# Justin900429/autonomous_driving_with_diffusion_model

Hardware: AMD Instinct MI355X
Metric: denoising-steps/sec (higher is better)
Workload: dtype f32

## Files before the change

autonomous_driving_with_diffusion_model_amd/_lib.py:

```python
from __future__ import annotations

import ctypes as C
import os
from typing import Optional, Sequence

import torch

_HERE = os.path.dirname(os.path.abspath(__file__))
LIB_PATH = os.environ.get("ADX_LIB") or os.path.join(_HERE, "libadx.so")

c_f32p = C.POINTER(C.c_float)
i32, i64, f32, vp = C.c_int32, C.c_int64, C.c_float, C.c_void_p


class TConvDesc(C.Structure):
    _fields_ = [("kind", i32), ("taps", i32), ("stride", i32), ("pad", i32), ("c0", i32), ("c1", i32),
                ("cout", i32), ("lin", i32), ("lout", i32), ("groups", i32), ("eps", f32), ("w_layout", i32),
                ("w_flip", i32), ("exact", i32), ("lin_valid", i32), ("lout_valid", i32)]


class TConvIO(C.Structure):
    _fields_ = [("x0", vp), ("x0_sb", i64), ("x0_sc", i64), ("x0_sl", i64),
                ("x1", vp), ("x1_sb", i64), ("x1_sc", i64), ("x1_sl", i64),
                ("packed_w", vp), ("bias", vp), ("gamma", vp), ("beta", vp),
# ... 121 lines not shown
    "adx_conv2d_packed_bytes": (C.c_size_t, [C.POINTER(Conv2dDesc)]),
    "adx_conv2d_pack": (i32, [C.POINTER(Conv2dDesc), vp, vp, vp]),
    "adx_conv2d_forward": (i32, [C.POINTER(Conv2dDesc), vp, vp, vp, vp, vp, vp, i32, i32, i32, i32, vp]),
    "adx_conv2d_cells_supported": (i32, [C.POINTER(Conv2dDesc), i32, i32, i32]),
    "adx_conv2d_forward_cells": (i32, [C.POINTER(Conv2dDesc), vp, vp, vp, vp, vp, vp, i32, i32, i32, i32, i32, vp]),
    "adx_conv2d_stem_pool": (i32, [vp, i32, vp, vp, vp, vp, vp, vp, i32, i32, i32, i32, vp]),
    "adx_conv2d_wgrad_scratch_bytes": (C.c_size_t, []),
    "adx_conv2d_wgrad": (i32, [C.POINTER(Conv2dDesc), vp, vp, vp, i32, i32, i32, vp, vp]),
    "adx_conv2d_wgrad_ex": (i32, [C.POINTER(Conv2dDesc), vp, vp, vp, i32, i32, i32, vp, i32, vp]),
    "adx_conv2d_wgrad_cells": (i32, [C.POINTER(Conv2dDesc), vp, vp, vp, vp, i32, i32, i32, vp, vp]),
    "adx_trajpred_create": (i32, [i32, C.POINTER(vp)]),
    "adx_trajpred_destroy": (None, [vp]),
    "adx_trajpred_num_params": (i32, [vp]),
    "adx_trajpred_packed_bytes": (C.c_size_t, [vp]),
    "adx_trajpred_scratch_bytes": (C.c_size_t, [vp, i32, i32]),
    "adx_trajpred_set_scratch": (i32, [vp, vp, C.c_size_t]),
    "adx_trajpred_pack": (i32, [vp, C.POINTER(vp), i32, vp, vp, vp]),
    "adx_trajpred_forward": (i32, [vp, vp, vp, i64, i64, vp, vp, i32, i32, vp]),
    "adx_trajpred_backward": (i32, [vp, vp, vp, i64, i64, vp, vp, vp, i32, i32, vp]),
    "adx_trajpred_backward_params": (i32, [vp, vp, vp, i64, i64, vp, vp, vp, vp, vp, i32, i32, C.c_float, C.c_uint64, vp]),
    "adx_trajpred_forward_train": (i32, [vp, vp, vp, i64, i64, vp, vp, i32, i32, C.c_float, C.c_uint64, vp]),
    "adx_trajpred_param_offsets": (i32, [vp, C.POINTER(i64), i32]),
    "adx_guided_output": (i32, [vp, vp, vp, vp, vp, f32, f32, vp, vp, i32, i32, vp]),
    "adx_optim_chunk": (i32, []),
    "adx_adamw_ema_step": (i32, [vp, vp, vp, i32, f32, f32, f32, f32, f32, i32, f32, i32, i32, vp]),
    "adx_adamw_ema_step_scaled": (i32, [vp, vp, vp, i32, f32, f32, f32, f32, f32, i32, f32, i32, i32, f32, vp]),
    "adx_image_normalize": (i32, [vp, vp, i32, i32, i32, C.POINTER(C.c_float), C.POINTER(C.c_float), vp]),
    "adx_probe_mfma_fp16": (i32, [vp, vp, i32, i32, C.POINTER(C.c_double), vp]),
    "adx_probe_mfma_fp16_16x16x32": (i32, [vp, vp, i32, i32, C.POINTER(C.c_double), vp]),
    "adx_image_augment": (i32, [vp, vp, i32, i32, i32, vp, vp, vp, vp, i32, vp]),
    "adx_ddim_step": (i32, [C.POINTER(StepCoef), vp, vp, vp, vp, vp, vp, vp, i32, i32, i32, vp]),
    "adx_ddpm_step": (i32, [C.POINTER(StepCoef), vp, vp, vp, vp, vp, vp, vp, i32, i32, i32, vp]),
    "adx_ddim_step_rng": (i32, [C.POINTER(StepCoef), vp, vp, vp, i32, i64, vp, vp, vp, vp, i32, i32, i32, vp]),
    "adx_ddpm_step_rng": (i32, [C.POINTER(StepCoef), vp, vp, vp, i32, i64, vp, vp, vp, vp, i32, i32, i32, vp]),
    "adx_dpm_step": (i32, [C.POINTER(DpmCoef), vp, vp, vp, vp, vp, i32, i32, i32, vp]),
    "adx_traj_select": (i32, [C.POINTER(SelectCfg), vp, vp, vp, vp, vp, vp]),
    "adx_control_state_bytes": (C.c_size_t, [i32, i32, i32]),
    "adx_control_step": (i32, [C.POINTER(ControlCfg), vp, vp, vp, vp, vp, vp]),
    "adx_control_reset": (i32, [vp, i32, i32, i32, vp, vp]),
    "adx_noise_normal": (i32, [vp, i32, i64, vp, i64, vp]),
    "adx_noise_words": (i32, [vp, i32, i64, vp, i64, vp]),
    "adx_noise_advance": (i32, [vp, vp]),
    "adx_warm_init": (i32, [vp, i32, vp, vp, i32, i32, i32, i32, f32, f32, vp, i64, i32, vp]),
    "adx_add_noise": (i32, [vp, vp, vp, vp, vp, i32, vp, i32, i32, i32, i32, vp]),
}

_LAZY_SIGS = {
    "adx_conv2d_pack_ds": (i32, [i32, i32, vp, vp, vp]),
    "adx_conv2d_block_s2_cells": (i32, [i32, i32, vp, vp, vp, vp, vp, vp, vp, vp, vp, i32, i32, i32, i32, vp]),
    "adx_ddim_step_pin": (i32, [C.POINTER(StepCoef), vp, vp, vp, vp, i32, i64, C.POINTER(PinDesc), vp, vp, i32, i32, i32, vp]),
    "adx_ddpm_step_pin": (i32, [C.POINTER(StepCoef), vp, vp, vp, vp, i32, i64, C.POINTER(PinDesc), vp, vp, i32, i32, i32, vp]),
    "adx_dpm_step_pin": (i32, [C.POINTER(DpmCoef), vp, vp, vp, vp, i32, i64, C.POINTER(PinDesc), vp, vp, i32, i32, i32, vp]),
    "adx_pin_apply": (i32, [vp, C.POINTER(PinDesc), vp, i64, i32, i32, i32, vp]),
}

EXPORTED_SYMBOLS = tuple(_SIGS) + tuple(_LAZY_SIGS)

_lib: Optional[C.CDLL] = None


class AdxError(RuntimeError):
    pass


class AdxRangeError(AdxError):

    def __init__(self, groups):
        self.groups = list(groups)
        super().__init__(f"values outside the fp16 range of the split kernels (|x| >= 65504 or NaN) in {', '.join(self.groups)}; "
                         "ADX_CHECK_RANGE=1 names the first tensor, ADX_CONV_EXACT=1 runs the perception pass on the exact-fp32 kernels")


def lib() -> C.CDLL:
    global _lib
    if _lib is None:
        if not os.path.exists(LIB_PATH):
            raise AdxError(
                f"{LIB_PATH} not found: the HIP extension is not built. Run `python -c 'import __graft_entry__ as g; "
                f"g.build()'` (or autonomous_driving_with_diffusion_model_amd/csrc/build.sh). There is no CPU fallback.")
        handle = C.CDLL(LIB_PATH)
        for name, (res, args) in _SIGS.items():
            fn = getattr(handle, name)
            fn.restype = res
            fn.argtypes = args
        _lib = handle
    return _lib


def lazy(name: str):
    handle = lib()
    res, args = _LAZY_SIGS[name]
    try:
        fn = getattr(handle, name)
    except AttributeError:
        raise AdxError(f"{LIB_PATH} does not export {name} (a library built from older sources?)") from None
    fn.restype = res
    fn.argtypes = args
    return fn


class NativeTape:

    def __init__(self, create, destroy, what: str):
        import weakref
        h = vp()
        check(create(C.byref(h)), what)
# ... 54 lines not shown
```

autonomous_driving_with_diffusion_model_amd/csrc/conv2d.hip:

```cpp
#include <stdlib.h>

#include <vector>

#include "adx_common.h"
#include "conv2d_internal.h"

namespace adx {

constexpr int kCoutT = 64;
constexpr size_t kMaxLds = 96 * 1024;

template <int STRIDE, int K, int ROWS, int CCH = 16>
__global__ void __launch_bounds__(256) conv2d_kernel(const Conv2dArgs a) {
  constexpr int TH = 4 * ROWS;
  constexpr int CC = (K == 7) ? 4 : CCH;
  constexpr int PH = (TH - 1) * STRIDE + K;
  constexpr int PW = (kTileW - 1) * STRIDE + K;
  constexpr int PLANE = PH * PW;
  constexpr int NP = CC * PLANE;
  constexpr int PITEMS = (NP + 255) / 256;
  constexpr int NTAPS = K * K;
  constexpr int NW4 = NTAPS * CC * (kCoutT / 4);
  constexpr int WITEMS = (NW4 + 255) / 256;
  extern __shared__ __attribute__((aligned(16))) float smem[];
// ... 430 lines not shown
  else if (L.stride == 2 && L.k == 7) conv2d_kernel<2, 7, 1><<<g, blk, lds, s>>>(a);
  else if (L.stride == 1 && L.k == 1) conv2d_kernel<1, 1, 1><<<g, blk, lds, s>>>(a);
  else {
    set_error("conv2d: no kernel for k=%d stride=%d (ResNet-34 uses 3x3 s1, 3x3 s2, 1x1 s2, 7x7 s2)", L.k, L.stride);
    return ADX_ERR_INVALID;
  }
  ADX_LAUNCH_CHECK();
  return ADX_OK;
}

}

using namespace adx;

static int spec_from_desc(const adx_conv2d_desc* d, ConvSpec* L) {
  ADX_REQUIRE(d != nullptr, "conv2d: null descriptor");
  ADX_REQUIRE(d->cin >= 1 && d->cout >= 64 && d->cout % kCoutT == 0, "conv2d: cout %d must be a multiple of %d", d->cout,
              kCoutT);
  ADX_REQUIRE(d->k >= 1 && d->k <= 7 && (d->stride == 1 || d->stride == 2) && d->pad >= 0 && d->pad <= 3,
              "conv2d: unsupported k/stride/pad %d/%d/%d", d->k, d->stride, d->pad);
  memset(L, 0, sizeof(*L));
  L->cin = d->cin; L->cout = d->cout; L->k = d->k; L->stride = d->stride; L->pad = d->pad;
  L->cc = d->cin >= 16 ? 16 : 4;
  L->cin_pad = round_up(d->cin, L->cc);
  return ADX_OK;
}

extern "C" {

size_t adx_conv2d_packed_bytes(const adx_conv2d_desc* d) {
  ConvSpec L;
  if (spec_from_desc(d, &L) != ADX_OK) return 0;
  return sizeof(float) * (conv2d_hs_eligible(L) ? conv2d_packed_floats(L) : (size_t)L.k * L.k * L.cin_pad * L.cout);
}

int adx_conv2d_pack(const adx_conv2d_desc* d, const float* w, float* packed, adx_stream stream) {
  ConvSpec L;
  int rc = spec_from_desc(d, &L);
  if (rc != ADX_OK) return rc;
  ADX_REQUIRE(w && packed, "adx_conv2d_pack: null pointer");
  return conv2d_pack_spec(L, w, packed, 0, (hipStream_t)stream);
}

int adx_conv2d_forward(const adx_conv2d_desc* d, const float* x, const float* packed_w, const float* scale,
                       const float* shift, const float* res, float* y, int32_t n, int32_t h, int32_t w, int32_t relu,
                       adx_stream stream) {
  ConvSpec L;
  int rc = spec_from_desc(d, &L);
  if (rc != ADX_OK) return rc;
  ADX_REQUIRE(x && packed_w && y, "adx_conv2d_forward: null tensor");
  ADX_REQUIRE((scale == nullptr) == (shift == nullptr), "adx_conv2d_forward: scale and shift go together");
  ADX_REQUIRE(n >= 1 && h + 2 * d->pad >= d->k && w + 2 * d->pad >= d->k, "adx_conv2d_forward: input too small");
  return conv2d_launch_raw(L, x, packed_w, scale, shift, res, y, n, h, w, relu, (hipStream_t)stream);
}

int adx_conv2d_cells_supported(const adx_conv2d_desc* d, int32_t n, int32_t h, int32_t w) {
  ConvSpec L;
  if (d == nullptr || spec_from_desc(d, &L) != ADX_OK) return 0;
  return conv2d_hs3x3_plain(L, n, h, w) ? 1 : 0;
}

int adx_conv2d_forward_cells(const adx_conv2d_desc* d, const void* x, const float* packed_w, const float* scale,
                             const float* shift, const void* res, void* y, int32_t n, int32_t h, int32_t w, int32_t relu,
                             int32_t fmt, adx_stream stream) {
  ConvSpec L;
  int rc = spec_from_desc(d, &L);
  if (rc != ADX_OK) return rc;
  ADX_REQUIRE(x && packed_w && y, "adx_conv2d_forward_cells: null tensor");
  ADX_REQUIRE((scale == nullptr) == (shift == nullptr), "adx_conv2d_forward_cells: scale and shift go together");
  ADX_REQUIRE(fmt >= 0 && fmt <= 7 && (fmt & kFmtYCells), "adx_conv2d_forward_cells: fmt %d (the output is a cell tensor)", fmt);
  ADX_REQUIRE(conv2d_hs3x3_plain(L, n, h, w), "adx_conv2d_forward_cells: not a plain launch of the pipelined 3x3 kernel "
              "(adx_conv2d_cells_supported)");
  return conv2d_launch_raw(L, (const float*)x, packed_w, scale, shift, (const float*)res, (float*)y, n, h, w, relu,
                           (hipStream_t)stream, nullptr, 0, nullptr, 0, nullptr, fmt);
}

static int block_s2_specs(int32_t cin, int32_t cout, ConvSpec* c1, ConvSpec* ds, const char* who) {
  const adx_conv2d_desc d1{cin, cout, 3, 2, 1}, dd{cin, cout, 1, 2, 0};
  int rc = spec_from_desc(&d1, c1);
  if (rc == ADX_OK) rc = spec_from_desc(&dd, ds);
  if (rc != ADX_OK) return rc;
  ADX_REQUIRE(resnet_fuses_ds(*c1, *ds), "%s: %d -> %d is no block entry the split-fp16 kernels fuse (cin %% 16, cout %% 64, not ADX_CONV_EXACT=1)",
              who, cin, cout);
  return ADX_OK;
}

int adx_conv2d_pack_ds(int32_t cin, int32_t cout, const float* w, float* packed, adx_stream stream) {
  ConvSpec c1, ds;
  const int rc = block_s2_specs(cin, cout, &c1, &ds, "adx_conv2d_pack_ds");
  if (rc != ADX_OK) return rc;
  ADX_REQUIRE(w && packed, "adx_conv2d_pack_ds: null pointer");
  return conv2d_hs_pack(ds, w, packed, 0, (hipStream_t)stream);
}

int adx_conv2d_block_s2_cells(int32_t cin, int32_t cout, const void* x, const float* packed_w1, const float* scale1, const float* shift1,
                              void* y1, const float* packed_wd, const float* scaled, const float* shiftd, void* yd, int32_t n, int32_t h,
                              int32_t w, int32_t flags, adx_stream stream) {
  ConvSpec c1, ds;
  const int rc = block_s2_specs(cin, cout, &c1, &ds, "adx_conv2d_block_s2_cells");
  if (rc != ADX_OK) return rc;
  ADX_REQUIRE(x && packed_w1 && y1 && packed_wd && yd, "adx_conv2d_block_s2_cells: null tensor");
  ADX_REQUIRE((scale1 == nullptr) == (shift1 == nullptr) && (scaled == nullptr) == (shiftd == nullptr),
              "adx_conv2d_block_s2_cells: scale and shift go together");
  ADX_REQUIRE(n >= 1 && h >= 1 && w >= 1 && flags >= 0 && flags <= 1, "adx_conv2d_block_s2_cells: bad shape %d x %d x %d or flags %d", n, h, w, flags);
  ADX_REQUIRE((size_t)n * cin * h * w * sizeof(float) < 0xC0000000u, "adx_conv2d_block_s2_cells: the input exceeds the 32-bit byte offsets");
  return conv2d_hs_launch_block_s2(c1, ds, (const float*)x, packed_w1, scale1, shift1, (float*)y1, packed_wd, scaled, shiftd, (float*)yd, n, h, w,
// ... 455 lines not shown
```

autonomous_driving_with_diffusion_model_amd/csrc/conv2d_hs16.hip:

```cpp
#include "adx_common.h"
#include "conv2d_internal.h"
#include "conv2d_hs_common.h"

namespace adx {

namespace {

typedef __attribute__((address_space(3))) void lds_void;

__device__ __forceinline__ f32x4 mfma16(f16x8 a, f16x8 b, f32x4 c) { return __builtin_amdgcn_mfma_f32_16x16x32_f16(a, b, c, 0, 0, 0); }

__device__ __forceinline__ void half4(uint32_t h0, uint32_t h1, uint32_t l0, uint32_t l1, float* out) {
  const float inv = 1.f / kLoScale;
  asm("v_fma_mix_f32 %0, %1, %2, %3 op_sel:[0,0,0] op_sel_hi:[1,0,1]" : "=v"(out[0]) : "v"(l0), "s"(inv), "v"(h0));
  asm("v_fma_mix_f32 %0, %1, %2, %3 op_sel:[1,0,1] op_sel_hi:[1,0,1]" : "=v"(out[1]) : "v"(l0), "s"(inv), "v"(h0));
  asm("v_fma_mix_f32 %0, %1, %2, %3 op_sel:[0,0,0] op_sel_hi:[1,0,1]" : "=v"(out[2]) : "v"(l1), "s"(inv), "v"(h1));
  asm("v_fma_mix_f32 %0, %1, %2, %3 op_sel:[1,0,1] op_sel_hi:[1,0,1]" : "=v"(out[3]) : "v"(l1), "s"(inv), "v"(h1));
}

}

template <bool DMA, int TRAIN = 0>
__global__ void __launch_bounds__(kQNT, 2) conv2d_hs3x3q_kernel(const Conv2dArgs a) {
  constexpr bool S2 = TRAIN == 3;
  static_assert(!S2 || DMA, "the stride-2 block entry stages with LDS-DMA only");
  constexpr int NT = kQNT, PW = kQPW, PLANE = DMA ? kQPlaneD : kQPlane, PP = DMA ? kQPlaneD : kQPlaneP, PIT = kQPit, WST = kQWst;
  constexpr int NPAIRS = DMA ? kQPairsD : kQPairs;
  constexpr int GST = DMA ? PP : 2 * PP, PLST = DMA ? 4 * PP : PP;
  extern __shared__ __attribute__((aligned(16))) unsigned char smem_raw[];
  u32x4* patch = reinterpret_cast<u32x4*>(smem_raw);
  u32x4* wl = patch + 2 * 8 * PP;
  float* ss = reinterpret_cast<float*>(wl + 2 * WST);
  u32x4* dummy = reinterpret_cast<u32x4*>(ss + 256);
  float* bsl = reinterpret_cast<float*>(dummy + 2);
  uint32_t* gnext = reinterpret_cast<uint32_t*>(bsl + 512);
  uint32_t* gpl = gnext + PIT * NT;
  const int tid = threadIdx.x, lane = tid & 63;
  const int wave = __builtin_amdgcn_readfirstlane(tid >> 6);
  const int rowpair = wave & 3, slab = wave >> 2;
  const int j = lane & 15, kq = lane >> 4;
  const int Qs = a.q_slots;
  const int xcd = blockIdx.x & 7, rr_ = blockIdx.x >> 3;
  const int ct = rr_ % a.cout_tiles, slot = rr_ / a.cout_tiles;
  const int nsp = a.tiles_x * a.tiles_y;
  const int sp_end = (int)(((long)(xcd + 1) * nsp) >> 3);
  int sp = (int)(((long)xcd * nsp) >> 3) + slot;
  if (sp >= sp_end) return;
  int ty = sp / a.tiles_x, tx = sp - ty * a.tiles_x;
  int oy0 = ty * kQTH, vx0 = tx * 32;
  auto vdiv = [&](int v) { return (int)(((float)v + 0.5f) * a.inv_vw); };
  const size_t hw = (size_t)a.H * a.W;
  const int nch16 = a.cin_pad / 16, nch32 = a.cin_pad / 32, nstages = nch32 * 9;
  constexpr uint32_t kOutside = 0xC0000000u;
  const __amdgpu_buffer_rsrc_t xrsrc = __builtin_amdgcn_make_buffer_rsrc(
      const_cast<float*>(a.x), 0, (int)(uint32_t)((size_t)a.N * a.Cin * hw * sizeof(float)), 0x00020000);
  const uint32_t plane_bytes = (uint32_t)(hw * sizeof(float));
  auto goff_of = [&](int t_, int k, int oy0_, int vx0_) -> uint32_t {
    const int e = t_ + NT * k;
    const int g = e / PLANE, p = e - g * PLANE;
    const int py = p / PW, px = p - py * PW;
    const int iy = oy0_ - 1 + py;
    const int v = vx0_ - 1 + px;
    const int ni = vdiv(v < 0 ? 0 : v);
    const int ix = v - ni * a.vw;
    const bool ok = e < NPAIRS && p < kQPlane && iy >= 0 && iy < a.H && ix >= 0 && ix < a.W && ni < a.N;
    return !ok ? kOutside : (uint32_t)((size_t)ni * a.Cin * hw * sizeof(float) + (size_t)g * 8 * hw * sizeof(float) + ((size_t)iy * a.W + ix) * 16);
  };
  auto goff_s2 = [&](int t_, int k, int oy0_, int vx0_, int pr, int pc) -> uint32_t {
    const int e = t_ + NT * k;
    const int g = e / PLANE, p = e - g * PLANE;
    const int py = p / PW, px = p - py * PW;
    const int q = oy0_ - 1 + py;
    const int v = vx0_ - 1 + px;
    const int ni = vdiv(v < 0 ? 0 : v);
    const int pcl = v - ni * a.vw;
    const int iy = 2 * q + pr, ix = 2 * pcl + pc;
    const bool ok = e < NPAIRS && py + pr > 0 && py <= kQTH && px + pc > 0 && px < PW - 1 && q >= 0 && iy < a.H && pcl >= 0 && pcl < a.OW &&
                    ix < a.W && ni < a.N;
    return !ok ? kOutside : (uint32_t)((size_t)ni * a.Cin * hw * sizeof(float) + (size_t)g * 8 * hw * sizeof(float) + ((size_t)iy * a.W + ix) * 16);
  };
  constexpr int kTap[9] = {1, 7, 4, 3, 5, 0, 2, 6, 8};
  uint32_t goff[PIT];
  int pcell[PIT];
#pragma unroll
  for (int k = 0; k < PIT; ++k) {
    const int e = tid + NT * k;
    const int g = e / PLANE, p = e - g * PLANE;
    if constexpr (S2) goff[k] = goff_s2(tid, k, oy0, vx0, 1, 0);
    else goff[k] = goff_of(tid, k, oy0, vx0);
    pcell[k] = e < NPAIRS ? g * GST + p : -1;
  }
  const u32x4* wsrc = reinterpret_cast<const u32x4*>(a.w);
  int wsrc_off[2];
// ... 38 lines not shown
      __builtin_amdgcn_raw_ptr_buffer_load_lds(wdrsrc, (lds_void*)(wl + set * WST + wcell + NT * k), 16, (uint32_t)(tid * 16),
                                               (uint32_t)(((ct * 2 + k) * nch16 + chunk * 2) * 256 * 16), 0, 0);
  };
  auto store_w = [&](int set, int buf) {
    if constexpr (!DMA) {
#pragma unroll
      for (int k = 0; k < 2; ++k) wl[buf * WST + tid + NT * k] = wv[set][k];
    }
  };
  auto load_p_at = [&](int chunk, int k, int set, uint32_t go) {
    const uint32_t cbase = (uint32_t)chunk * 32u * plane_bytes;
    if constexpr (DMA) {
      if (k < PIT - 1 || wcell + NT * k < NPAIRS) {
        u32x4* d = patch + set * 8 * PP + wcell + NT * k;
        __builtin_amdgcn_raw_ptr_buffer_load_lds(xrsrc, (lds_void*)d, 16, go, cbase, 0, 0);
        __builtin_amdgcn_raw_ptr_buffer_load_lds(xrsrc, (lds_void*)(d + PLST), 16, go, cbase + 4 * plane_bytes, 0, 0);
      }
    } else {
      pvh[set] = __builtin_amdgcn_raw_buffer_load_b128(xrsrc, go, cbase, 0);
      pvl[set] = __builtin_amdgcn_raw_buffer_load_b128(xrsrc, go, cbase + 4 * plane_bytes, 0);
    }
  };
  auto load_p = [&](int chunk, int k, int set) { load_p_at(chunk, k, set, goff[k]); };
  auto store_p = [&](int set, int k, int buf) {
    if constexpr (!DMA) {
      u32x4* pd = patch + buf * 8 * PP + pcell[k];
      u32x4* d0 = (k < PIT - 1 || pcell[k] >= 0) ? pd : dummy;
      u32x4* d1 = (k < PIT - 1 || pcell[k] >= 0) ? pd + PP : dummy + 1;
      *d0 = pvh[set];
      *d1 = pvl[set];
    }
  };


  if constexpr (S2) load_w_tap(0, kTap[0], 0);
  else load_w(0, 0);
  store_w(0, 0);
#pragma unroll
  for (int k = 0; k < PIT; ++k) { load_p(0, k, 0); store_p(0, k, 0); }
  if constexpr (!DMA) load_w(1, 1);
  if (tid < 256) ss[tid] = ssv;
  if constexpr (TRAIN == 2) {
    const int which = tid >> 7, c = ct * 128 + (tid & 127);
    const float mu = a.bs_mean[c], rs = a.bs_rstd[c];
    const float sc = a.bs_gamma[c] * rs;
    bsl[tid] = which == 0 ? mu : (which == 1 ? rs : (which == 2 ? sc : __builtin_fmaf(-mu, sc, a.bs_beta[c])));
  }
  if constexpr (S2) {
    if (tid < 256) {
      const int c = ct * 128 + (tid & 127);
      bsl[tid] = a.scale_ds == nullptr ? (tid < 128 ? 1.f : 0.f) : (tid < 128 ? a.scale_ds[c] : a.shift_ds[c]);
    }
  }
  if constexpr (DMA) asm volatile("s_waitcnt vmcnt(0)" ::: "memory");
  __syncthreads();

  bool bad = false;
  for (;;) {
  int zero_ = 0;
  asm volatile("" : "+s"(zero_));
  const int tl = tid + zero_;
  if constexpr (DMA) {
    if constexpr (!S2) {
#pragma unroll
      for (int k = 0; k < PIT; ++k) goff[k] = goff_of(tl, k, oy0, vx0);
    }
#pragma unroll
    for (int k = 0; k < 2; ++k) {
      const int e = tl + NT * k;
      const int sl = e >> 9, half16 = (e >> 8) & 1, within = e & 255;
      wsrc_off[k] = (((ct * 2 + sl) * nch16 + half16) * 9) * 256 + within;
    }
  }
  const int j_l = tl & 15, kq_l = (tl & 63) >> 4;
  const int pb_lane = kq_l * GST + (rowpair * 2) * PW + j_l;
  const int wa_lane = slab * 512 + (kq_l >> 1) * 256 + (kq_l & 1) * 64 + j_l;
  const int sp_next = sp + Qs;
  const bool has_next = DMA && sp_next < sp_end;
  const int nty = sp_next / a.tiles_x, ntx = sp_next - nty * a.tiles_x;
  const int n_oy0 = nty * kQTH, n_vx0 = ntx * 32;
  if constexpr (S2) {
#pragma unroll
    for (int k = 0; k < PIT; ++k) {
      const uint32_t g10 = goff_s2(tl, k, oy0, vx0, 1, 0);
      gpl[(0 * PIT + k) * NT + tid] = goff_s2(tl, k, oy0, vx0, 1, 1);
      gpl[(1 * PIT + k) * NT + tid] = g10;
      gpl[(2 * PIT + k) * NT + tid] = goff_s2(tl, k, oy0, vx0, 0, 1);
      gpl[(3 * PIT + k) * NT + tid] = goff_s2(tl, k, oy0, vx0, 0, 0);
      gnext[k * NT + tid] = has_next ? goff_s2(tl, k, n_oy0, n_vx0, 1, 0) : g10;
    }
  } else if constexpr (DMA) {
#pragma unroll
    for (int k = 0; k < PIT; ++k) gnext[k * NT + tid] = has_next ? goff_of(tl, k, n_oy0, n_vx0) : goff[k];
  }
#pragma unroll
  for (int cb = 0; cb < 4; ++cb)
#pragma unroll
    for (int pb = 0; pb < 4; ++pb)
#pragma unroll
      for (int i = 0; i < 4; ++i) { accm[cb][pb][i] = 0.f; accl[cb][pb][i] = 0.f; }

  auto s2_stage = [&](const u32x4* pb0, const u32x4* wa0) {
    __builtin_amdgcn_sched_barrier(0);
    f16x8 A[2][4], B[2][4];
#pragma unroll
    for (int pl = 0; pl < 2; ++pl) {
#pragma unroll
      for (int cb = 0; cb < 4; ++cb) A[pl][cb] = __builtin_bit_cast(f16x8, wa0[pl * 128 + cb * 16]);
#pragma unroll
      for (int pb = 0; pb < 4; ++pb) B[pl][pb] = __builtin_bit_cast(f16x8, pb0[pl * PLST + (pb >> 1) * PW + (pb & 1) * 16]);
    }
#pragma unroll
    for (int pb = 0; pb < 4; ++pb) {
#pragma unroll
      for (int cb = 0; cb < 4; ++cb) {
        accm[cb][pb] = mfma16(A[0][cb], B[0][pb], accm[cb][pb]);
        accl[cb][pb] = mfma16(A[0][cb], B[1][pb], accl[cb][pb]);
      }
#pragma unroll
      for (int cb = 0; cb < 4; ++cb) accl[cb][pb] = mfma16(A[1][cb], B[0][pb], accl[cb][pb]);
    }
    asm volatile("s_waitcnt vmcnt(0)" ::: "memory");
    __syncthreads();
  };
  if constexpr (S2) {
    constexpr int kBuf[9] = {0, 0, 1, 0, 0, 1, 1, 1, 1};
    constexpr int kPlaneNext[9] = {3, 3, 2, 0, 0, 1, 1, 1, 1};
    constexpr int kRound0[9] = {0, 2, 0, 0, 2, 0, 1, 2, 3}, kRounds[9] = {2, 1, 3, 2, 1, 1, 1, 1, 0};
    for (int cp = 0; cp < nch32; cp += 2) {
#pragma unroll
      for (int i = 0; i < 18; ++i) {
        const int cpar = i / 9, t = i % 9, c = cp + cpar, kh = kTap[t] / 3, kw = kTap[t] % 3;
        const bool last = cpar == 1 && c + 1 >= nch32;
        if (t < 8) load_w_tap(c, kTap[t + 1], (i + 1) & 1);
        else if (!last) load_w_tap(c + 1, kTap[0], (i + 1) & 1);
        else load_w_ds(0, 0);
        const int nplane = t >= 5 && last ? 3 : kPlaneNext[t];
        const int nchunk = t < 5 ? c : (last ? 0 : c + 1);
#pragma unroll
        for (int k = kRound0[t]; k < kRound0[t] + kRounds[t]; ++k) load_p_at(nchunk, k, kBuf[t] ^ 1, gpl[(nplane * PIT + k) * NT + tid]);
        s2_stage(patch + kBuf[t] * 8 * PP + pb_lane + (kh > 0) * PW + (kw > 0), wl + (i & 1) * WST + wa_lane);
      }
    }
  } else
  for (int cp = 0; cp < nch32; cp += 2) {
#pragma unroll
    for (int i = 0; i < 18; ++i) {
      const int s = 9 * cp + i;
      const int cpar = i / 9, t = i % 9, kh = t / 3, kw = t % 3;
      const u32x4* pb0 = patch + cpar * 8 * PP + pb_lane + kh * PW + kw;
      const u32x4* wa0 = wl + (i & 1) * WST + wa_lane;
      if constexpr (DMA) {
        load_w(s + 1 < nstages ? s + 1 : (has_next ? 0 : nstages - 1), (i + 1) & 1);
        if (kw == 0) {
          if (cpar == 0 || cp + cpar + 1 < nch32) load_p(cp + cpar + 1, kh, (cpar + 1) & 1);
          else load_p_at(has_next ? 0 : nch32 - 1, kh, (cpar + 1) & 1, gnext[kh * NT + tid]);
        }
      } else {
        load_w(s + 2 < nstages ? s + 2 : nstages - 1, i & 1);
        if (kw == 0) load_p(cp + cpar + 1 < nch32 ? cp + cpar + 1 : nch32 - 1, kh, i & 1);
      }
      __builtin_amdgcn_sched_barrier(0);
      f16x8 A[2][4], B[2][4];
#pragma unroll
      for (int pl = 0; pl < 2; ++pl) {
#pragma unroll
        for (int cb = 0; cb < 4; ++cb) A[pl][cb] = __builtin_bit_cast(f16x8, wa0[pl * 128 + cb * 16]);
#pragma unroll
        for (int pb = 0; pb < 4; ++pb) B[pl][pb] = __builtin_bit_cast(f16x8, pb0[pl * PLST + (pb >> 1) * PW + (pb & 1) * 16]);
      }
      auto row_mfmas = [&](int rr) {
#pragma unroll
        for (int pb = 2 * rr; pb < 2 * rr + 2; ++pb) {
#pragma unroll
          for (int cb = 0; cb < 4; ++cb) {
            accm[cb][pb] = mfma16(A[0][cb], B[0][pb], accm[cb][pb]);
            accl[cb][pb] = mfma16(A[0][cb], B[1][pb], accl[cb][pb]);
          }
#pragma unroll
          for (int cb = 0; cb < 4; ++cb) accl[cb][pb] = mfma16(A[1][cb], B[0][pb], accl[cb][pb]);
          if (pb == 0) {
            store_w((i + 1) & 1, (i + 1) & 1);
            if (kw == 1) store_p((i + 1) & 1, kh, (cpar + 1) & 1);
          }
        }
      };
      row_mfmas(0);
      row_mfmas(1);
      if constexpr (DMA) asm volatile("s_waitcnt vmcnt(0)" ::: "memory");
      __syncthreads();
    }
  }

  if constexpr (TRAIN == 2) {
    const float xs_inv = reinterpret_cast<const float*>(a.x_amax)[1];
    const uint32_t plane_ob = (uint32_t)(a.OH * a.OW) * (uint32_t)sizeof(float);
    const uint32_t bplane = (uint32_t)(a.OH * a.OW);
    const uint32_t img_bytes = (uint32_t)a.N * (uint32_t)a.Cout * plane_ob, bit_bytes = (uint32_t)a.N * (uint32_t)(a.Cout >> 3) * bplane;
    const int rw = kq;
    const int vcol = vx0 + 16 * (rw & 1) + j;
    const int nl = vdiv(vcol), xl = vcol - nl * a.vw;
    const bool col_valid = nl < a.N && xl < a.W;
    const bool mask_bits = a.bs_mask == 1, res_masked = a.res_bits != nullptr;
    const __amdgpu_buffer_rsrc_t yrsrc = __builtin_amdgcn_make_buffer_rsrc(a.y, 0, (int)img_bytes, 0x00020000);
    const __amdgpu_buffer_rsrc_t rrsrc = __builtin_amdgcn_make_buffer_rsrc(
        const_cast<float*>(a.res != nullptr ? a.res : a.y), 0, a.res != nullptr ? (int)img_bytes : 0, 0x00020000);
    const __amdgpu_buffer_rsrc_t wrsrc = __builtin_amdgcn_make_buffer_rsrc(const_cast<float*>(a.bs_raw), 0, (int)img_bytes, 0x00020000);
    const __amdgpu_buffer_rsrc_t brsrc = __builtin_amdgcn_make_buffer_rsrc(
        const_cast<uint8_t*>(mask_bits ? a.bs_bits : reinterpret_cast<const uint8_t*>(a.y)), 0, mask_bits ? (int)bit_bytes : 0, 0x00020000);
    const __amdgpu_buffer_rsrc_t qrsrc = __builtin_amdgcn_make_buffer_rsrc(
        const_cast<uint8_t*>(res_masked ? a.res_bits : reinterpret_cast<const uint8_t*>(a.y)), 0, res_masked ? (int)bit_bytes : 0, 0x00020000);
    const int cout0 = ct * 128 + slab * 64;
    const float* bsw = bsl + slab * 64 + 8 * (rw >> 1);
    float* red = reinterpret_cast<float*>(patch + 8 * PP);
    uint32_t voff[2], boff[2];
    bool valid[2];
#pragma unroll
    for (int rr = 0; rr < 2; ++rr) {
      const int oy = oy0 + rowpair * 2 + rr;
      valid[rr] = col_valid && oy < a.OH;
      voff[rr] = valid[rr] ? (uint32_t)nl * (uint32_t)a.Cout * plane_ob + (uint32_t)(oy * a.OW + xl) * 4u + (uint32_t)(8 * (rw >> 1)) * plane_ob : kOutside;
      boff[rr] = valid[rr] ? (uint32_t)nl * (uint32_t)(a.Cout >> 3) * bplane + (uint32_t)(oy * a.OW + xl) + (uint32_t)(rw >> 1) * bplane : kOutside;
    }
    float dmx = 0.f;
#pragma unroll
    for (int cb = 0; cb < 4; ++cb) {
      float sm[8], sq[8];
#pragma unroll
      for (int c8 = 0; c8 < 8; ++c8) { sm[c8] = 0.f; sq[c8] = 0.f; }
#pragma unroll
      for (int rr = 0; rr < 2; ++rr) {
        float o[8], res8[8], rw8[8];
#pragma unroll
        for (int c8 = 0; c8 < 8; ++c8) {
          const uint32_t so = (uint32_t)(cout0 + 16 * cb + c8) * plane_ob;
          res8[c8] = u2f(__builtin_amdgcn_raw_buffer_load_b32(rrsrc, voff[rr], so, 0));
          rw8[c8] = u2f(__builtin_amdgcn_raw_buffer_load_b32(wrsrc, voff[rr], so, 0));
        }
        const uint32_t bso = (uint32_t)((cout0 >> 3) + 2 * cb) * bplane;
        const uint32_t mres = res_masked ? (uint32_t)__builtin_amdgcn_raw_buffer_load_b8(qrsrc, boff[rr], bso, 0) : 0xFFu;
        const uint32_t mbs = mask_bits ? (uint32_t)__builtin_amdgcn_raw_buffer_load_b8(brsrc, boff[rr], bso, 0) : 0u;
#pragma unroll
        for (int i = 0; i < 4; ++i) {
// ... 116 lines not shown
        }
    }
  } else {
  int pass = 0;
  do {
  if constexpr (S2) {
    if (pass == 1) {
#pragma unroll
      for (int cb = 0; cb < 4; ++cb)
#pragma unroll
        for (int pb = 0; pb < 4; ++pb)
#pragma unroll
          for (int i = 0; i < 4; ++i) { accm[cb][pb][i] = 0.f; accl[cb][pb][i] = 0.f; }
      for (int d = 0; d < nch32; d += 2) {
#pragma unroll
        for (int i = 0; i < 2; ++i) {
          const int c = d + i;
          if (i == 0 || c + 1 < nch32) {
            load_w_ds(c + 1, (i + 1) & 1);
#pragma unroll
            for (int k = 0; k < PIT; ++k) load_p_at(c + 1, k, (i + 1) & 1, gpl[(3 * PIT + k) * NT + tid]);
          } else {
            load_w_tap(0, kTap[0], 0);
#pragma unroll
            for (int k = 0; k < PIT; ++k) load_p_at(0, k, 0, gnext[k * NT + tid]);
          }
          s2_stage(patch + i * 8 * PP + pb_lane + PW + 1, wl + i * WST + wa_lane);
        }
      }
    }
  }
  float* const yout = S2 && pass == 1 ? a.y_ds : a.y;
  const float* const ssp = S2 && pass == 1 ? bsl : ss;
  const int relu = S2 && pass == 1 ? 0 : a.relu;
  const int rw = kq;
  const int vcol = vx0 + 16 * (rw & 1) + j;
  const int nl = vdiv(vcol), xl = vcol - nl * a.vw;
  const bool col_valid = nl < a.N && xl < (S2 ? a.OW : a.W);
  const uint32_t plane_ob = (uint32_t)(a.OH * a.OW) * (uint32_t)sizeof(float);
  const uint32_t cplane = (uint32_t)(a.OH * a.OW) * 16u;
  const uint32_t img_bytes = (uint32_t)a.N * (uint32_t)a.Cout * plane_ob;
  const uint32_t img_off = (uint32_t)nl * (uint32_t)a.Cout * plane_ob;
  const __amdgpu_buffer_rsrc_t yrsrc = __builtin_amdgcn_make_buffer_rsrc(yout, 0, (int)img_bytes, 0x00020000);
  const __amdgpu_buffer_rsrc_t rrsrc = __builtin_amdgcn_make_buffer_rsrc(
      const_cast<float*>(a.res != nullptr ? a.res : a.y), 0, a.res != nullptr ? (int)img_bytes : 0, 0x00020000);
  const int cout0 = ct * 128 + slab * 64;
  const uint32_t cell0 = (uint32_t)(cout0 >> 3) * 2u * cplane;
  uint32_t vcell[2];
#pragma unroll
  for (int rr = 0; rr < 2; ++rr) {
    const int oy = oy0 + rowpair * 2 + rr;
    vcell[rr] = (col_valid && oy < a.OH) ? img_off + (uint32_t)(oy * a.OW + xl) * 16u + (uint32_t)(rw >> 1) * 2u * cplane : kOutside;
  }
  u32x4 rh[4][2], rl[4][2];
#pragma unroll
  for (int cb = 0; cb < 4; ++cb)
#pragma unroll
    for (int rr = 0; rr < 2; ++rr) {
      const uint32_t so = cell0 + (uint32_t)(2 * cb) * 2u * cplane;
      if constexpr (S2) {
        rh[cb][rr] = u32x4{0u, 0u, 0u, 0u};
        rl[cb][rr] = u32x4{0u, 0u, 0u, 0u};
      } else {
        rh[cb][rr] = __builtin_amdgcn_raw_buffer_load_b128(rrsrc, vcell[rr], so, 0);
        rl[cb][rr] = __builtin_amdgcn_raw_buffer_load_b128(rrsrc, vcell[rr], so + cplane, 0);
      }
    }
  const float* sc = ssp + slab * 64;
  const float* sh = ssp + 128 + slab * 64;
  float am[2] = {0.f, 0.f};
#pragma unroll
  for (int cb = 0; cb < 4; ++cb)
#pragma unroll
    for (int rr = 0; rr < 2; ++rr) {
      float x[4], y[4];
#pragma unroll
      for (int i = 0; i < 4; ++i) {
        const int cl = cb * 16 + 4 * kq + i;
        x[i] = (accm[cb][2 * rr][i] + accl[cb][2 * rr][i] * (1.f / kLoScale)) * sc[cl] + sh[cl];
        y[i] = (accm[cb][2 * rr + 1][i] + accl[cb][2 * rr + 1][i] * (1.f / kLoScale)) * sc[cl] + sh[cl];
      }
      float o[8];
#pragma unroll
      for (int i = 0; i < 4; ++i) {
        const auto sw = __builtin_amdgcn_permlane16_swap(f2u(x[i]), f2u(y[i]), false, false);
        o[i] = u2f(sw[0]);
        o[4 + i] = u2f(sw[1]);
      }
      float r8[8];
      half4(rh[cb][rr][0], rh[cb][rr][1], rl[cb][rr][0], rl[cb][rr][1], r8);
      half4(rh[cb][rr][2], rh[cb][rr][3], rl[cb][rr][2], rl[cb][rr][3], r8 + 4);
#pragma unroll
      for (int i = 0; i < 8; ++i) {
        const float tsum = o[i] + r8[i];
        o[i] = relu ? __builtin_fmaxf(tsum, 0.f) : tsum;
        am[rr] = fp16_amax(am[rr], o[i]);
      }
      u32x4 hi, lo;
      split8(o, 1.f, hi, lo);
      const uint32_t so = cell0 + (uint32_t)(2 * cb) * 2u * cplane;
      __builtin_amdgcn_raw_buffer_store_b128(hi, yrsrc, vcell[rr], so, 0);
      __builtin_amdgcn_raw_buffer_store_b128(lo, yrsrc, vcell[rr], so + cplane, 0);
      asm volatile("s_nop 0" ::"v"(hi), "v"(lo));
    }
  bad |= ((vcell[0] != kOutside) & out_of_fp16(am[0])) | ((vcell[1] != kOutside) & out_of_fp16(am[1]));
  } while (S2 && ++pass < 2);
  }
  if (!has_next) break;
  if constexpr (TRAIN == 1 || TRAIN == 2) __syncthreads();
  sp = sp_next; tx = ntx; ty = nty; oy0 = n_oy0; vx0 = n_vx0;
  }
  range_flag(a.status, bad);
}

int conv2d_hs3x3q_launch(const Hs3x3Plan& p, Conv2dArgs a, hipStream_t s) {
  typedef void (*QKernel)(const Conv2dArgs);
  static const QKernel table[2][3] = {
      {&conv2d_hs3x3q_kernel<false, 0>, &conv2d_hs3x3q_kernel<false, 1>, &conv2d_hs3x3q_kernel<false, 2>},
      {&conv2d_hs3x3q_kernel<true, 0>, &conv2d_hs3x3q_kernel<true, 1>, &conv2d_hs3x3q_kernel<true, 2>}};
  static std::atomic<uint64_t> attr{0};
  if (DeviceOnce once{attr}; once) {
    for (int dma = 0; dma < 2; ++dma)
      for (const QKernel k : table[dma])
        ADX_CHECK_HIP(hipFuncSetAttribute(reinterpret_cast<const void*>(k), hipFuncAttributeMaxDynamicSharedMemorySize, (int)(dma ? kQLdsD : kQLds)));
    once.commit();
  }
  ADX_REQUIRE((long)a.N * p.vw < (1L << 21), "conv2d_hs: batch x width exceeds the virtual-row arithmetic");
  const size_t tiles = (size_t)p.cout_tiles * p.tiles_x * p.tiles_y;
  ADX_REQUIRE(tiles < (1u << 31), "conv2d_hs: grid too large");
  ADX_REQUIRE((size_t)a.N * a.Cout * a.OH * a.OW * sizeof(float) < 0xC0000000u && (size_t)a.N * a.Cin * a.H * a.W * sizeof(float) < 0xC0000000u,
              "conv2d_hs: a cell-layout tensor exceeds the 32-bit byte offsets");
  a.vw = p.vw; a.inv_vw = 1.f / (float)p.vw;
  a.tiles_x = p.tiles_x; a.tiles_y = p.tiles_y; a.cout_tiles = p.cout_tiles; a.ntiles = (int)tiles;
  a.q_slots = p.q_slots;
  a.ksplit = p.ksplit; a.cper = p.cper; a.part = nullptr;
  table[p.dma][p.stats]<<<dim3((unsigned)p.grid), dim3(p.threads), p.lds, s>>>(a);
  ADX_LAUNCH_CHECK();
  return ADX_OK;
}

int conv2d_hs3x3q_s2_launch(const HsS2Plan& p, Conv2dArgs a, hipStream_t s) {
  static std::atomic<uint64_t> attr{0};
  if (DeviceOnce once{attr}; once) {
    ADX_CHECK_HIP(hipFuncSetAttribute(reinterpret_cast<const void*>(&conv2d_hs3x3q_kernel<true, 3>), hipFuncAttributeMaxDynamicSharedMemorySize, (int)kQLdsS2));
    once.commit();
  }
  ADX_REQUIRE(p.q && a.x_cells && a.y_cells && a.w_ds != nullptr && a.y_ds != nullptr && a.res == nullptr && a.x_amax == nullptr,
              "conv2d_hs: the 16x16x32 block entry takes a cell input, two cell outputs, no residual and no dynamic range");
  a.vw = p.vw; a.inv_vw = 1.f / (float)p.vw;
  a.tiles_x = p.tiles_x; a.tiles_y = p.tiles_y; a.cout_tiles = p.cout_tiles; a.ntiles = p.cout_tiles * p.tiles_x * p.tiles_y;
  a.q_slots = p.q_slots;
  a.ksplit = 1; a.cper = a.cin_pad / kHsCC; a.part = nullptr;
  conv2d_hs3x3q_kernel<true, 3><<<dim3((unsigned)p.grid), dim3(p.threads), p.lds, s>>>(a);
  ADX_LAUNCH_CHECK();
  return ADX_OK;
}

}
```

include/adx.h:

```cpp
#ifndef ADX_H
#define ADX_H

#include <stddef.h>
#include <stdint.h>

#ifdef __cplusplus
extern "C" {
#endif

#define ADX_OK 0
#define ADX_ERR_INVALID (-1)
#define ADX_ERR_HIP (-2)
#define ADX_ERR_STATE (-3)
#define ADX_ERR_RANGE (-4)

typedef void* adx_stream;

int adx_version(void);
const char* adx_source_hash(void);
const char* adx_last_error(void);


typedef struct adx_tconv_desc {
  int32_t kind, taps, stride, pad;
// ... 96 lines not shown
size_t adx_unet_train_workspace_bytes(const adx_unet* u, int32_t rows);
int adx_unet_forward_train(adx_unet* u, const void* packed, void* workspace, size_t workspace_bytes,
                           const adx_unet_io* io, adx_unet_tape* tape, adx_stream s);
int adx_unet_backward(adx_unet* u, const void* packed, void* workspace, size_t workspace_bytes, adx_unet_tape* tape,
                      const float* d_out, const float* d_time_embed ,
                      float* d_img_feature, const float* const* params, float* const* grads, int32_t n_grads,
                      adx_stream s);
int adx_gn_mish_backward(const float* dy, int64_t dy_sb, int64_t dy_sc, int64_t dy_sl, const float* pre,
                         const float* stats, const float* gamma, const float* beta, float* dc, float* dgamma,
                         float* dbeta, float* dbias, float* dtb, int64_t dtb_stride, int32_t B, int32_t C, int32_t L,
                         int32_t groups, adx_stream s);
int adx_tconv_wgrad(const adx_tconv_desc* d, const adx_tconv_io* io, const float* dc, float* dw, adx_stream s);
int adx_bias_grad(const float* dc, float* db, int32_t B, int32_t C, int32_t L, adx_stream s);
int adx_chan_layernorm_forward(const float* x, int64_t sb, int64_t sc, int64_t sl, const float* g, const float* b, float* xn,
                               float* mean, float* rstd, int32_t B, int32_t C, int32_t L, int32_t L_valid, adx_stream s);
int adx_chan_layernorm_backward(const float* dy, const float* x, int64_t sb, int64_t sc, int64_t sl, const float* mean,
                                const float* rstd, const float* g, float* dx, float* dg, float* db, int32_t B, int32_t C,
                                int32_t L, int32_t L_valid, int32_t accumulate, adx_stream s);
int adx_linattn_forward(const float* qkv, float* o, int32_t B, int32_t L, int32_t L_valid, adx_stream s);
int adx_linattn_backward(const float* qkv, const float* dout, float* dqkv, int32_t B, int32_t L, int32_t L_valid, adx_stream s);

typedef struct adx_resnet adx_resnet;
int adx_resnet_create(int32_t out_dim, adx_resnet** out);
void adx_resnet_destroy(adx_resnet* r);
int adx_resnet_num_tensors(const adx_resnet* r);
size_t adx_resnet_packed_bytes(const adx_resnet* r);
int adx_resnet_pack(adx_resnet* r, const float* const* tensors, int32_t n, void* packed, adx_stream s);
size_t adx_resnet_workspace_bytes(const adx_resnet* r, int32_t batch, int32_t h, int32_t w);
int adx_resnet_forward(adx_resnet* r, const void* packed, void* workspace, const float* img ,
                       int32_t batch, int32_t h, int32_t w, float* feature , adx_stream s);
int adx_resnet_forward_u8(adx_resnet* r, const void* packed, void* workspace, const uint8_t* frames_hwc,
                          const float* mean , const float* stdv , int32_t batch, int32_t h, int32_t w,
                          float* feature , adx_stream s);
#define ADX_RESNET_PLAN_INTS 24
#define ADX_RESNET_PLAN_CAPTURING 1
enum { ADX_RESNET_PLAN_STEM_POOL = 0, ADX_RESNET_PLAN_STEM = 1, ADX_RESNET_PLAN_MAXPOOL = 2, ADX_RESNET_PLAN_CONV = 3,
       ADX_RESNET_PLAN_ENTRY = 4, ADX_RESNET_PLAN_AVGPOOL_FC = 5 };
int adx_resnet_plan_describe(const adx_resnet* r, int32_t batch, int32_t h, int32_t w, int32_t flags, int32_t* n_records, int32_t* ints,
                             int32_t max_records);
int32_t adx_resnet_status_words(const adx_resnet* r);
int adx_resnet_set_status(adx_resnet* r, uint32_t* words );
const char* adx_resnet_status_name(const adx_resnet* r, int32_t group);

typedef struct adx_conv2d_desc { int32_t cin, cout, k, stride, pad; } adx_conv2d_desc;
size_t adx_conv2d_packed_bytes(const adx_conv2d_desc* d);
int adx_conv2d_pack(const adx_conv2d_desc* d, const float* w , float* packed, adx_stream s);
int adx_conv2d_forward(const adx_conv2d_desc* d, const float* x, const float* packed_w, const float* scale,
                       const float* shift, const float* res, float* y, int32_t n, int32_t h, int32_t w,
                       int32_t relu, adx_stream s);
int adx_conv2d_cells_supported(const adx_conv2d_desc* d, int32_t n, int32_t h, int32_t w);
int adx_conv2d_forward_cells(const adx_conv2d_desc* d, const void* x, const float* packed_w, const float* scale,
                             const float* shift, const void* res, void* y, int32_t n, int32_t h, int32_t w, int32_t relu,
                             int32_t fmt, adx_stream s);
int adx_conv2d_pack_ds(int32_t cin, int32_t cout, const float* w, float* packed, adx_stream s);
int adx_conv2d_block_s2_cells(int32_t cin, int32_t cout, const void* x, const float* packed_w1, const float* scale1,
                              const float* shift1, void* y1, const float* packed_wd, const float* scaled, const float* shiftd,
                              void* yd, int32_t n, int32_t h, int32_t w, int32_t flags, adx_stream s);
int adx_conv2d_stem_pool(const void* x, int32_t x_u8, const float* packed_w, const float* scale, const float* shift,
                         const float* mean, const float* stdv, void* y, int32_t n, int32_t h, int32_t w, int32_t y_cells,
                         adx_stream s);
size_t adx_conv2d_wgrad_scratch_bytes(void);
int adx_conv2d_wgrad(const adx_conv2d_desc* d, const float* x, const float* dy, float* dw, int32_t n, int32_t h,
                     int32_t w, void* scratch, adx_stream s);
int adx_conv2d_wgrad_ex(const adx_conv2d_desc* d, const float* x, const float* dy, float* dw, int32_t n, int32_t h,
                        int32_t w, void* scratch, int32_t estimate_range, adx_stream s);
int adx_conv2d_wgrad_cells(const adx_conv2d_desc* d, const void* x_cells, const void* dy_cells, const float* dy_scale, float* dw,
                           int32_t n, int32_t h, int32_t w, void* scratch, adx_stream s);

typedef struct adx_resnet_tape adx_resnet_tape;
int adx_resnet_tape_create(adx_resnet_tape** out);
void adx_resnet_tape_destroy(adx_resnet_tape* t);
size_t adx_resnet_train_workspace_bytes(const adx_resnet* r, int32_t batch, int32_t h, int32_t w);
int adx_resnet_forward_train(adx_resnet* r, const float* const* tensors, int32_t n_tensors, void* packed,
                             void* workspace, size_t workspace_bytes, const float* img, int32_t batch, int32_t h,
                             int32_t w, float* feature, adx_resnet_tape* tape, int32_t update_running, adx_stream s);
int adx_resnet_backward(adx_resnet* r, const float* const* tensors, float* const* grads, int32_t n_tensors,
                        void* workspace, size_t workspace_bytes, adx_resnet_tape* tape, const float* d_feature,
                        adx_stream s);
int32_t adx_resnet_backward_groups(const adx_resnet* r);
int32_t adx_resnet_tensor_group(const adx_resnet* r, int32_t tensor);
int adx_resnet_backward_events(adx_resnet* r, const float* const* tensors, float* const* grads, int32_t n_tensors,
                               void* workspace, size_t workspace_bytes, adx_resnet_tape* tape, const float* d_feature,
                               void* const* events, int32_t n_events, adx_stream s);
int32_t adx_resnet_bn_layers(const adx_resnet* r);
int32_t adx_resnet_bn_tensor(const adx_resnet* r, int32_t layer);
int adx_resnet_forward_train_ex(adx_resnet* r, const float* const* tensors, int32_t n_tensors, void* packed,
                                void* workspace, size_t workspace_bytes, const float* img, int32_t batch, int32_t h,
                                int32_t w, float* feature, adx_resnet_tape* tape, int32_t update_running, uint64_t frozen_bn,
                                adx_stream s);
int adx_resnet_backward_ex(adx_resnet* r, const float* const* tensors, float* const* grads, int32_t n_tensors,
                           void* workspace, size_t workspace_bytes, adx_resnet_tape* tape, const float* d_feature,
                           uint64_t frozen_bn, void* const* events, int32_t n_events, adx_stream s);
int adx_resnet_tape_describe(const adx_resnet_tape* tape, const void* workspace, int32_t index, int32_t* n_records,
                             int32_t* ints, int64_t* offs);

typedef struct adx_trajpred adx_trajpred;
int adx_trajpred_create(int32_t out_dim, adx_trajpred** out);
void adx_trajpred_destroy(adx_trajpred* t);
int adx_trajpred_num_params(const adx_trajpred* t);
size_t adx_trajpred_packed_bytes(const adx_trajpred* t);
size_t adx_trajpred_scratch_bytes(const adx_trajpred* t, int32_t batch, int32_t T);
int adx_trajpred_set_scratch(adx_trajpred* t, void* scratch, size_t bytes);
int adx_trajpred_pack(adx_trajpred* t, const float* const* params, int32_t n, const float* freqs, void* packed,
                      adx_stream s);
int adx_trajpred_forward(adx_trajpred* t, const void* packed, const float* action, int64_t act_sb, int64_t act_st,
                         const float* time_embed, float* out, int32_t batch, int32_t T, adx_stream s);
// ... 148 lines not shown
```

Before: 172.1.

## Defer next-tile offset computation into the pipeline and specialize epilogue branches

In the DMA non-training 3x3 half-split conv kernel, the next tile's gather offsets are now computed lazily inside the main loop, right before the cross-tile prefetch. The current offsets are reloaded from the LDS gnext buffer instead of being recomputed at the top of each tile, with gnext initialized before the loop. The epilogue is templated on relu and residual via std::true_type/false_type so each variant is compiled without runtime branches. Also adds an optional compile-time timestamp tracing facility and an adx_conv2d_set_status export.

Measured after the change: 175.6 (median of 6 runs). 1.02x the previous value.

```diff
diff --git a/autonomous_driving_with_diffusion_model_amd/_lib.py b/autonomous_driving_with_diffusion_model_amd/_lib.py
--- a/autonomous_driving_with_diffusion_model_amd/_lib.py
+++ b/autonomous_driving_with_diffusion_model_amd/_lib.py
@@ -197,6 +197,7 @@
     "adx_ddpm_step_pin": (i32, [C.POINTER(StepCoef), vp, vp, vp, vp, i32, i64, C.POINTER(PinDesc), vp, vp, i32, i32, i32, vp]),
     "adx_dpm_step_pin": (i32, [C.POINTER(DpmCoef), vp, vp, vp, vp, i32, i64, C.POINTER(PinDesc), vp, vp, i32, i32, i32, vp]),
     "adx_pin_apply": (i32, [vp, C.POINTER(PinDesc), vp, i64, i32, i32, i32, vp]),
+    "adx_conv2d_set_status": (i32, [vp]),
 }
 
 EXPORTED_SYMBOLS = tuple(_SIGS) + tuple(_LAZY_SIGS)
diff --git a/autonomous_driving_with_diffusion_model_amd/csrc/conv2d.hip b/autonomous_driving_with_diffusion_model_amd/csrc/conv2d.hip
--- a/autonomous_driving_with_diffusion_model_amd/csrc/conv2d.hip
+++ b/autonomous_driving_with_diffusion_model_amd/csrc/conv2d.hip
@@ -506,6 +506,11 @@
   ADX_REQUIRE((scale == nullptr) == (shift == nullptr), "adx_conv2d_forward: scale and shift go together");
   ADX_REQUIRE(n >= 1 && h + 2 * d->pad >= d->k && w + 2 * d->pad >= d->k, "adx_conv2d_forward: input too small");
   return conv2d_launch_raw(L, x, packed_w, scale, shift, res, y, n, h, w, relu, (hipStream_t)stream);
+}
+
+int adx_conv2d_set_status(uint32_t* word) {
+  conv2d_set_status(word);
+  return ADX_OK;
 }
 
 int adx_conv2d_cells_supported(const adx_conv2d_desc* d, int32_t n, int32_t h, int32_t w) {
diff --git a/autonomous_driving_with_diffusion_model_amd/csrc/conv2d_hs16.hip b/autonomous_driving_with_diffusion_model_amd/csrc/conv2d_hs16.hip
--- a/autonomous_driving_with_diffusion_model_amd/csrc/conv2d_hs16.hip
+++ b/autonomous_driving_with_diffusion_model_amd/csrc/conv2d_hs16.hip
@@ -1,3 +1,4 @@
+#include <type_traits>
 #include "adx_common.h"
 #include "conv2d_internal.h"
 #include "conv2d_hs_common.h"
@@ -17,6 +18,18 @@
   asm("v_fma_mix_f32 %0, %1, %2, %3 op_sel:[0,0,0] op_sel_hi:[1,0,1]" : "=v"(out[2]) : "v"(l1), "s"(inv), "v"(h1));
   asm("v_fma_mix_f32 %0, %1, %2, %3 op_sel:[1,0,1] op_sel_hi:[1,0,1]" : "=v"(out[3]) : "v"(l1), "s"(inv), "v"(h1));
 }
+
+#ifdef ADX_HSQ_TRACE
+constexpr int kHsqBlocks = 1024, kHsqTiles = 8, kHsqWords = 8 + 8 * kHsqTiles;
+__device__ unsigned long long g_hsq_trace[kHsqBlocks * kHsqWords];
+#define HSQ_ON (DMA && TRAIN == 0)
+#define HSQ_STAMP(word, v) do { if constexpr (HSQ_ON) { if (threadIdx.x == 0) hsq_lds[word] = (v); } } while (0)
+#define HSQ_TRACE(word) HSQ_STAMP(word, __builtin_amdgcn_s_memtime())
+#define HSQ_TRACE_TILE(slot) do { if (trace_tile < kHsqTiles) HSQ_TRACE(8 + 8 * trace_tile + (slot)); } while (0)
+#else
+#define HSQ_TRACE(word)
+#define HSQ_TRACE_TILE(slot)
+#endif
 
 }
 
@@ -39,6 +52,15 @@
   const int wave = __builtin_amdgcn_readfirstlane(tid >> 6);
   const int rowpair = wave & 3, slab = wave >> 2;
   const int j = lane & 15, kq = lane >> 4;
+#ifdef ADX_HSQ_TRACE
+  __shared__ unsigned long long hsq_lds[kHsqWords];
+  int trace_tile = 0;
+  if constexpr (HSQ_ON) {
+    if (tid < 64) { hsq_lds[tid] = 0; if (tid + 64 < kHsqWords) hsq_lds[tid + 64] = 0; }
+  }
+  HSQ_TRACE(0);
+  HSQ_STAMP(2, __builtin_amdgcn_s_memrealtime());
+#endif
   const int Qs = a.q_slots;
   const int xcd = blockIdx.x & 7, rr_ = blockIdx.x >> 3;
   const int ct = rr_ % a.cout_tiles, slot = rr_ / a.cout_tiles;
@@ -183,16 +205,27 @@
       bsl[tid] = a.scale_ds == nullptr ? (tid < 128 ? 1.f : 0.f) : (tid < 128 ? a.scale_ds[c] : a.shift_ds[c]);
     }
   }
+  constexpr bool TURN = DMA && TRAIN == 0;
+  if constexpr (TURN) {
+    __builtin_assume(nch32 >= 2);
+#pragma unroll
+    for (int k = 0; k < PIT; ++k) gnext[k * NT + tid] = goff[k];
+  }
   if constexpr (DMA) asm volatile("s_waitcnt vmcnt(0)" ::: "memory");
   __syncthreads();
+  HSQ_TRACE(1);
 
   bool bad = false;
   for (;;) {
+  HSQ_TRACE_TILE(0);
   int zero_ = 0;
   asm volatile("" : "+s"(zero_));
   const int tl = tid + zero_;
   if constexpr (DMA) {
-    if constexpr (!S2) {
+    if constexpr (TURN) {
+#pragma unroll
+      for (int k = 0; k < PIT; ++k) goff[k] = gnext[k * NT + tid];
+    } else if constexpr (!S2) {
 #pragma unroll
       for (int k = 0; k < PIT; ++k) goff[k] = goff_of(tl, k, oy0, vx0);
     }
@@ -220,7 +253,7 @@
       gpl[(3 * PIT + k) * NT + tid] = goff_s2(tl, k, oy0, vx0, 0, 0);
       gnext[k * NT + tid] = has_next ? goff_s2(tl, k, n_oy0, n_vx0, 1, 0) : g10;
     }
-  } else if constexpr (DMA) {
+  } else if constexpr (DMA && !TURN) {
 #pragma unroll
     for (int k = 0; k < PIT; ++k) gnext[k * NT + tid] = has_next ? goff_of(tl, k, n_oy0, n_vx0) : goff[k];
   }
@@ -230,6 +263,7 @@
     for (int pb = 0; pb < 4; ++pb)
 #pragma unroll
       for (int i = 0; i < 4; ++i) { accm[cb][pb][i] = 0.f; accl[cb][pb][i] = 0.f; }
+  HSQ_TRACE_TILE(1);
 
   auto s2_stage = [&](const u32x4* pb0, const u32x4* wa0) {
     __builtin_amdgcn_sched_barrier(0);
@@ -285,7 +319,14 @@
         load_w(s + 1 < nstages ? s + 1 : (has_next ? 0 : nstages - 1), (i + 1) & 1);
         if (kw == 0) {
           if (cpar == 0 || cp + cpar + 1 < nch32) load_p(cp + cpar + 1, kh, (cpar + 1) & 1);
-          else load_p_at(has_next ? 0 : nch32 - 1, kh, (cpar + 1) & 1, gnext[kh * NT + tid]);
+          else if constexpr (TURN) {
+            if (has_next) {
+              int z_ = 0;
+              asm volatile("" : "+s"(z_));
+              gnext[kh * NT + tid] = goff_of(tid + z_, kh, n_oy0, n_vx0);
+            }
+            load_p_at(has_next ? 0 : nch32 - 1, kh, (cpar + 1) & 1, gnext[kh * NT + tid]);
+          } else load_p_at(has_next ? 0 : nch32 - 1, kh, (cpar + 1) & 1, gnext[kh * NT + tid]);
         }
       } else {
         load_w(s + 2 < nstages ? s + 2 : nstages - 1, i & 1);
@@ -320,6 +361,10 @@
       row_mfmas(1);
       if constexpr (DMA) asm volatile("s_waitcnt vmcnt(0)" ::: "memory");
       __syncthreads();
+#ifdef ADX_HSQ_TRACE
+      if (i == 0) { if (cp == 0) HSQ_TRACE_TILE(2); }
+      if (i == 17) { if (cp + 2 >= nch32) HSQ_TRACE_TILE(3); }
+#endif
     }
   }
 
@@ -542,6 +587,70 @@
     const int oy = oy0 + rowpair * 2 + rr;
     vcell[rr] = (col_valid && oy < a.OH) ? img_off + (uint32_t)(oy * a.OW + xl) * 16u + (uint32_t)(rw >> 1) * 2u * cplane : kOutside;
   }
+  if constexpr (TURN) {
+  float am[2];
+  auto epilogue = [&](auto relu_, auto with_res) {
+  u32x4 rh[4][2], rl[4][2];
+#pragma unroll
+  for (int cb = 0; cb < 4; ++cb)
+#pragma unroll
+    for (int rr = 0; rr < 2; ++rr) {
+      const uint32_t so = cell0 + (uint32_t)(2 * cb) * 2u * cplane;
+      if (with_res) {
+        rh[cb][rr] = __builtin_amdgcn_raw_buffer_load_b128(rrsrc, vcell[rr], so, 0);
+        rl[cb][rr] = __builtin_amdgcn_raw_buffer_load_b128(rrsrc, vcell[rr], so + cplane, 0);
+      }
+    }
+  const float* sc = ssp + slab * 64;
+  const float* sh = ssp + 128 + slab * 64;
+  am[0] = 0.f; am[1] = 0.f;
+#pragma unroll
+  for (int cb = 0; cb < 4; ++cb)
+#pragma unroll
+    for (int rr = 0; rr < 2; ++rr) {
+      float x[4], y[4];
+#pragma unroll
+      for (int i = 0; i < 4; ++i) {
+        const int cl = cb * 16 + 4 * kq + i;
+        x[i] = (accm[cb][2 * rr][i] + accl[cb][2 * rr][i] * (1.f / kLoScale)) * sc[cl] + sh[cl];
+        y[i] = (accm[cb][2 * rr + 1][i] + accl[cb][2 * rr + 1][i] * (1.f / kLoScale)) * sc[cl] + sh[cl];
+      }
+      float o[8];
+#pragma unroll
+      for (int i = 0; i < 4; ++i) {
+        const auto sw = __builtin_amdgcn_permlane16_swap(f2u(x[i]), f2u(y[i]), false, false);
+        o[i] = u2f(sw[0]);
+        o[4 + i] = u2f(sw[1]);
+      }
+      float r8[8];
+      if (with_res) {
+        half4(rh[cb][rr][0], rh[cb][rr][1], rl[cb][rr][0], rl[cb][rr][1], r8);
+        half4(rh[cb][rr][2], rh[cb][rr][3], rl[cb][rr][2], rl[cb][rr][3], r8 + 4);
+      } else {
+#pragma unroll
+        for (int i = 0; i < 8; ++i) r8[i] = 0.f;
+      }
+#pragma unroll
+      for (int i = 0; i < 8; ++i) {
+        const float tsum = o[i] + r8[i];
+        o[i] = relu_ ? __builtin_fmaxf(tsum, 0.f) : tsum;
+        am[rr] = fp16_amax(am[rr], o[i]);
+      }
+      u32x4 hi, lo;
+      split8(o, 1.f, hi, lo);
+      const uint32_t so = cell0 + (uint32_t)(2 * cb) * 2u * cplane;
+      __builtin_amdgcn_raw_buffer_store_b128(hi, yrsrc, vcell[rr], so, 0);
+      __builtin_amdgcn_raw_buffer_store_b128(lo, yrsrc, vcell[rr], so + cplane, 0);
+      asm volatile("s_nop 0" ::"v"(hi), "v"(lo));
+    }
+  };
+  constexpr std::true_type yes{};
+  constexpr std::false_type no{};
+  if (a.res != nullptr) { if (relu) epilogue(yes, yes); else epilogue(no, yes); }
+  else { if (relu) epilogue(yes, no); else epilogue(no, no); }
+  const bool out0 = out_of_fp16(am[0]), out1 = out_of_fp16(am[1]);
+  bad |= ((vcell[0] != kOutside) & out0) | ((vcell[1] != kOutside) & out1);
+  } else {
   u32x4 rh[4][2], rl[4][2];
 #pragma unroll
   for (int cb = 0; cb < 4; ++cb)
@@ -594,12 +703,28 @@
       asm volatile("s_nop 0" ::"v"(hi), "v"(lo));
     }
   bad |= ((vcell[0] != kOutside) & out_of_fp16(am[0])) | ((vcell[1] != kOutside) & out_of_fp16(am[1]));
+  }
   } while (S2 && ++pass < 2);
   }
+#ifdef ADX_HSQ_TRACE
+  HSQ_TRACE_TILE(4);
+  ++trace_tile;
+#endif
   if (!has_next) break;
   if constexpr (TRAIN == 1 || TRAIN == 2) __syncthreads();
   sp = sp_next; tx = ntx; ty = nty; oy0 = n_oy0; vx0 = n_vx0;
   }
+#ifdef ADX_HSQ_TRACE
+  HSQ_TRACE(4);
+  HSQ_STAMP(3, __builtin_amdgcn_s_memrealtime());
+  HSQ_STAMP(5, (unsigned long long)trace_tile);
+  if constexpr (HSQ_ON) {
+    if (tid < 64 && blockIdx.x < kHsqBlocks) {
+      g_hsq_trace[blockIdx.x * kHsqWords + tid] = hsq_lds[tid];
+      if (tid + 64 < kHsqWords) g_hsq_trace[blockIdx.x * kHsqWords + tid + 64] = hsq_lds[tid + 64];
+    }
+  }
+#endif
   range_flag(a.status, bad);
 }
 
@@ -647,3 +772,14 @@
 }
 
 }
+
+#ifdef ADX_HSQ_TRACE
+extern "C" int adx_hsq_trace_read(unsigned long long* host, int nwords) {
+  if (nwords < 0) {
+    void* d = nullptr;
+    if (const hipError_t e = hipGetSymbolAddress(&d, HIP_SYMBOL(adx::g_hsq_trace)); e != hipSuccess) return (int)e;
+    return (int)hipMemset(d, 0, sizeof(unsigned long long) * adx::kHsqBlocks * adx::kHsqWords);
+  }
+  return (int)hipMemcpyFromSymbol(host, HIP_SYMBOL(adx::g_hsq_trace), (size_t)nwords * 8);
+}
+#endif
diff --git a/include/adx.h b/include/adx.h
--- a/include/adx.h
+++ b/include/adx.h
@@ -172,6 +172,7 @@
 int adx_conv2d_forward_cells(const adx_conv2d_desc* d, const void* x, const float* packed_w, const float* scale,
                              const float* shift, const void* res, void* y, int32_t n, int32_t h, int32_t w, int32_t relu,
                              int32_t fmt, adx_stream s);
+int adx_conv2d_set_status(uint32_t* word );
 int adx_conv2d_pack_ds(int32_t cin, int32_t cout, const float* w, float* packed, adx_stream s);
 int adx_conv2d_block_s2_cells(int32_t cin, int32_t cout, const void* x, const float* packed_w1, const float* scale1,
                               const float* shift1, void* y1, const float* packed_wd, const float* scaled, const float* shiftd,
```
